# lpiccinelli-eth/UniDepth

Hardware: NVIDIA H100
Metric: images/sec UniDepthV2.infer ViT-L/14 480x640 (higher is better)
Workload: dtype f16 operands, f32 accumulate/residual

## Files before the change

### include/udb.h

```cpp
#ifndef UDB_H_
#define UDB_H_
#include <stddef.h>
#include <stdint.h>

#ifdef __cplusplus
extern "C" {
#endif

#define UDB_VERSION 1

int udb_version(void);

typedef struct udb_profile_entry_t {
  char name[48];
  float ms;
  double flops;
  double bytes;
} udb_profile_entry_t;
int udb_profile_begin(void* stream);
int udb_profile_end(udb_profile_entry_t* out, int32_t cap);
const char* udb_last_error(void);
int64_t udb_launch_count(void);

enum { UDB_A_MATRIX = 0, UDB_A_CONV3X3 = 1 };
// ... 5 lines not shown
  const void* w;
  int32_t M, N, K;
  int32_t lda, ldw;
  int32_t a_mode;
  int32_t conv_B, conv_H, conv_W, conv_C, conv_inH, conv_inW, conv_off, conv_TH, conv_TW;
  int32_t conv_cstride, conv_coff;
  const float* bias;
  const float* gamma;
  const void* resid;
  int32_t resid_f32;
  void* out;
  int32_t out_f32;
  void* out2;
  int32_t out2_leaky;
  int32_t act;
  int32_t store_mode;
  int64_t ldc;
  int32_t rows_per_group, group_stride, row_offset;
  int32_t resid_mod, resid_row_offset;
  int64_t ldr;
  int32_t ct_k, ct_cout, ct_h, ct_w, ct_pad;
  const float* head_w;
  float head_b, head_add;
  int32_t a_split_k;
  int32_t out_split;
  float* ln_stats_out;
  const float* ln_stats_in;
  const float* ln_c1;
  int32_t ln_parts, ln_part_cols;
  float ln_eps;
} udb_gemm_t;

int udb_gemm_f16(const udb_gemm_t* g, void* stream);

typedef struct udb_conv_halo_t {
  const void* x;
  const void* w;
  const float* bias;
  int32_t B, H, W, C, cstride, coff, cout, act;
  void* out;
  int64_t ldc;
  const float* head_w;
  float head_b, head_add;
  float* head_out;
} udb_conv_halo_t;
int udb_conv3x3_halo_f16(const udb_conv_halo_t* c, void* stream);

typedef struct udb_attn_t {
  const void* q;
  const void* k;
  const void* v;
  void* out;
  int32_t B, heads, seq_q, seq_k, head_dim;
  int32_t ldq, ldk, ldv, ldo;
  int32_t q_col0, k_col0, v_col0, o_col0;
  float scale;
  int32_t split;
  int32_t lo_off_q, lo_off_k, lo_off_v, lo_off_o;
} udb_attn_t;

int udb_attention_f16(const udb_attn_t* a, void* stream);

typedef struct udb_layernorm_t {
  const void* in;
  int32_t in_f32;
  void* out;
// ... 292 lines not shown
```

### unidepth_b200/_cabi.py

```python
from __future__ import annotations

import ctypes as C
import os

_HERE = os.path.dirname(os.path.abspath(__file__))
LIB_PATH = os.environ.get("UDB_LIB", os.path.join(_HERE, "libudb.so"))

A_MATRIX, A_CONV3X3 = 0, 1
ACT_NONE, ACT_GELU, ACT_LEAKY = 0, 1, 2
STORE_ROWS, STORE_CONVT, STORE_CONVTILE, STORE_HEAD = 0, 1, 2, 3

vp, i32, i64, f32 = C.c_void_p, C.c_int32, C.c_int64, C.c_float


class Gemm(C.Structure):
    _fields_ = [
        ("a", vp), ("w", vp), ("M", i32), ("N", i32), ("K", i32), ("lda", i32), ("ldw", i32),
        ("a_mode", i32),
        ("conv_B", i32), ("conv_H", i32), ("conv_W", i32), ("conv_C", i32), ("conv_inH", i32),
        ("conv_inW", i32), ("conv_off", i32), ("conv_TH", i32), ("conv_TW", i32),
        ("conv_cstride", i32), ("conv_coff", i32),
        ("bias", vp), ("gamma", vp), ("resid", vp), ("resid_f32", i32), ("out", vp), ("out_f32", i32),
        ("out2", vp), ("out2_leaky", i32), ("act", i32), ("store_mode", i32), ("ldc", i64),
        ("rows_per_group", i32), ("group_stride", i32), ("row_offset", i32),
# ... 125 lines not shown
        ("mean", vp), ("k4", vp), ("B", i32), ("net_h", i32), ("net_w", i32), ("pad_l", i32), ("pad_r", i32),
        ("pad_t", i32), ("pad_b", i32), ("H", i32), ("W", i32), ("out_depth", vp), ("out_points", vp),
    ]


class V1Config(C.Structure):
    _fields_ = [
        ("depths", i32 * 4), ("dims", i32 * 4), ("hidden", i32), ("heads", i32), ("expansion", i32),
        ("dec_depths", i32 * 3), ("encoder", i32), ("net_h", i32), ("net_w", i32),
    ]


class InferV1Args(C.Structure):
    _fields_ = [
        ("rgb", vp), ("rgb_is_u8", i32), ("scale255", i32), ("normalize", i32), ("B", i32), ("H", i32), ("W", i32),
        ("intrinsics", vp), ("skip_camera", i32), ("workspace", vp), ("workspace_bytes", C.c_size_t),
        ("out_intrinsics", vp), ("out_points", vp), ("out_depth", vp),
    ]


class ProfileEntry(C.Structure):
    _fields_ = [("name", C.c_char * 48), ("ms", f32), ("flops", C.c_double), ("bytes", C.c_double)]


DT_F16, DT_F32 = 0, 1

EXPORTS = {
    "udb_version": (i32, []),
    "udb_last_error": (C.c_char_p, []),
    "udb_launch_count": (i64, []),
    "udb_profile_begin": (i32, [vp]),
    "udb_profile_end": (i32, [C.POINTER(ProfileEntry), i32]),
    "udb_gemm_f16": (i32, [C.POINTER(Gemm), vp]),
    "udb_conv3x3_halo_f16": (i32, [C.POINTER(ConvHalo), vp]),
    "udb_attention_f16": (i32, [C.POINTER(Attn), vp]),
    "udb_layernorm": (i32, [C.POINTER(LayerNorm), vp]),
    "udb_preprocess_patchify": (i32, [C.POINTER(Preprocess), vp]),
    "udb_posembed_bicubic": (i32, [vp, i32, i32, vp, i32, i32, vp]),
    "udb_set_cls_rows": (i32, [vp, vp, vp, i32, i32, i32, vp]),
    "udb_set_cls_rows_ln": (i32, [vp, vp, vp, vp, vp, i32, i32, i32, i32, i32, vp]),
    "udb_small_linear_f32": (i32, [C.POINTER(SmallLinear), vp]),
    "udb_camera_attn4_f32": (i32, [vp, vp, vp, vp, i32, i32, i32, vp]),
    "udb_camera_intrinsics": (i32, [vp, i32, i32, i32, f32, i32, i32, vp, vp, vp, vp]),
    "udb_ray_embed": (i32, [C.POINTER(RayEmbed), vp]),
    "udb_upsample2x_nhwc_f16": (i32, [vp, vp, i32, i32, i32, i32, vp]),
    "udb_resize_ac_pad_nhwc_f16": (i32, [vp, vp, i32, i32, i32, i32, i32, i32, i32, vp]),
    "udb_reflect_pad1_nhwc_f16": (i32, [vp, vp, i32, i32, i32, i32, vp]),
    "udb_reflect_border_fill_nhwc_f16": (i32, [vp, i32, i32, i32, i32, vp]),
    "udb_postprocess": (i32, [C.POINTER(Postprocess), vp]),
    "udb_camera_adjust_k": (i32, [vp, i32, f32, i32, i32, vp, vp]),
    "udb_create": (i32, [C.POINTER(Config), C.POINTER(vp)]),
    "udb_destroy": (None, [vp]),
    "udb_set_weight": (i32, [vp, C.c_char_p, vp, C.POINTER(i64), i32, i32]),
    "udb_set_scalar": (i32, [vp, C.c_char_p, C.c_double]),
    "udb_geometry": (i32, [vp, i32, i32, i32, C.POINTER(Geometry)]),
    "udb_workspace_bytes": (C.c_size_t, [vp, i32, i32, i32, i32]),
    "udb_schedule_bytes": (C.c_size_t, [vp, i32, i32, i32, i32]),
    "udb_infer_v2": (i32, [vp, C.POINTER(InferArgs), vp]),
    "udb_v1_preprocess": (i32, [C.POINTER(V1Preprocess), vp]),
    "udb_layernorm_any": (i32, [C.POINTER(LayerNormAny), vp]),
    "udb_dwconv7_nhwc_f16": (i32, [vp, vp, vp, vp, i32, i32, i32, i32, vp]),
    "udb_max_accum_f16": (i32, [vp, vp, i64, i32, vp]),
    "udb_spatial_mean_f32": (i32, [vp, vp, i32, i32, i32, vp]),
    "udb_vit_tap": (i32, [vp, vp, vp, i32, i32, i32, i32, vp]),
    "udb_aa_resize_nhwc_f16": (i32, [vp, vp, i32, i32, i32, i32, i32, i32, vp]),
    "udb_v1_rays_sh81": (i32, [C.POINTER(V1Rays), vp]),
# ... 68 lines not shown
```

### unidepth_b200/csrc/common.cu

```cuda
#include "common.h"

#include <stdarg.h>
#include <stdlib.h>
#include <string.h>

#include <vector>

namespace udb {

static thread_local char g_err[512] = "";
std::atomic<int64_t> g_launches{0};

void set_error(const char* fmt, ...) {
  va_list ap;
  va_start(ap, fmt);
  vsnprintf(g_err, sizeof(g_err), fmt, ap);
  va_end(ap);
}

struct ProfEntry {
  const char* name;
  cudaEvent_t ev;
  double flops, bytes;
};
// ... 34 lines not shown
    per_dev[dev & 63].store(n, std::memory_order_relaxed);
  }
  return n;
}

bool pdl_enabled() {
  static const bool on = [] {
    const char* e = getenv("UDB_PDL");
    return e ? atoi(e) != 0 : true;
  }();
  return on;
}

typedef CUresult (*EncodeTiledFn)(CUtensorMap*, CUtensorMapDataType, cuuint32_t, void*,
                                  const cuuint64_t*, const cuuint64_t*, const cuuint32_t*,
                                  const cuuint32_t*, CUtensorMapInterleave, CUtensorMapSwizzle,
                                  CUtensorMapL2promotion, CUtensorMapFloatOOBfill);

static EncodeTiledFn get_encode() {
  static EncodeTiledFn fn = nullptr;
  if (!fn) {
    void* p = nullptr;
    cudaDriverEntryPointQueryResult q;
    cudaError_t e = cudaGetDriverEntryPoint("cuTensorMapEncodeTiled", &p, cudaEnableDefault, &q);
    if (e != cudaSuccess || q != cudaDriverEntryPointSuccess || !p) {
      set_error("cuTensorMapEncodeTiled entry point unavailable (%s)", cudaGetErrorString(e));
      return nullptr;
    }
    fn = reinterpret_cast<EncodeTiledFn>(p);
  }
  return fn;
}

int make_tmap_f16(CUtensorMap* map, const void* base, int rank, const uint64_t* dims,
                  const uint64_t* strides_bytes, const uint32_t* box, bool swizzle128) {
  EncodeTiledFn fn = get_encode();
  if (!fn) return 1;
  cuuint64_t gdim[5];
  cuuint64_t gstr[5];
  cuuint32_t bx[5];
  cuuint32_t es[5];
  for (int i = 0; i < rank; ++i) {
    gdim[i] = dims[i];
    bx[i] = box[i];
    es[i] = 1;
    if (i > 0) gstr[i - 1] = strides_bytes[i - 1];
  }
  if ((reinterpret_cast<uintptr_t>(base) & 15) != 0) {
    set_error("TMA base pointer %p is not 16-byte aligned", base);
    return 1;
  }
  for (int i = 0; i + 1 < rank; ++i) {
    if (gstr[i] % 16 != 0) {
      set_error("TMA stride %d = %llu bytes is not a multiple of 16", i, (unsigned long long)gstr[i]);
      return 1;
    }
  }
  CUresult r = fn(map, CU_TENSOR_MAP_DATA_TYPE_FLOAT16, (cuuint32_t)rank, const_cast<void*>(base),
                  gdim, gstr, bx, es, CU_TENSOR_MAP_INTERLEAVE_NONE,
                  swizzle128 ? CU_TENSOR_MAP_SWIZZLE_128B : CU_TENSOR_MAP_SWIZZLE_NONE,
                  CU_TENSOR_MAP_L2_PROMOTION_L2_256B, CU_TENSOR_MAP_FLOAT_OOB_FILL_NONE);
  if (r != CUDA_SUCCESS) {
    set_error("cuTensorMapEncodeTiled failed: CUresult %d (rank %d dims %llu,%llu box %u,%u)", (int)r,
              rank, (unsigned long long)dims[0], (unsigned long long)(rank > 1 ? dims[1] : 0), box[0],
              rank > 1 ? box[1] : 0);
    return 1;
  }
  return 0;
}

}

extern "C" {
int udb_version(void) { return UDB_VERSION; }
const char* udb_last_error(void) { return udb::g_err; }
int64_t udb_launch_count(void) { return udb::g_launches.load(); }

int udb_profile_begin(void* stream) {
  using namespace udb;
  if (g_prof_on) { set_error("udb_profile_begin: already profiling"); return 1; }
  g_prof.clear();
  g_prof_stream = reinterpret_cast<cudaStream_t>(stream);
  if (cudaEventCreate(&g_prof_start) != cudaSuccess || cudaEventRecord(g_prof_start, g_prof_stream) != cudaSuccess) {
    set_error("udb_profile_begin: event creation failed");
    return 1;
  }
  g_prof_on = true;
  return 0;
}

int udb_profile_end(udb_profile_entry_t* out, int32_t cap) {
  using namespace udb;
  if (!g_prof_on) { set_error("udb_profile_end: not profiling"); return -1; }
  g_prof_on = false;
// ... 24 lines not shown
```

### unidepth_b200/csrc/common.h

```cpp
#pragma once
#include <cuda.h>
#include <cuda_runtime.h>
#include <stdint.h>
#include <stdio.h>

#include <atomic>

#include "../../include/udb.h"

namespace udb {

void set_error(const char* fmt, ...);
extern std::atomic<int64_t> g_launches;

int check_launch(const char* what);
void note_work(double flops, double bytes);

int num_sms();

inline bool first_on_device(std::atomic<uint64_t>& mask) {
  int d = 0;
  cudaGetDevice(&d);
  const uint64_t bit = 1ull << (d & 63);
  return !(mask.fetch_or(bit) & bit);
}

bool pdl_enabled();

template <typename Kernel, typename... Args>
inline cudaError_t launch_ex(Kernel kernel, dim3 grid, dim3 block, size_t smem, cudaStream_t st, int cluster_x,
                             Args... args) {
  cudaLaunchConfig_t cfg{};
  cfg.gridDim = grid;
  cfg.blockDim = block;
  cfg.dynamicSmemBytes = smem;
  cfg.stream = st;
  cudaLaunchAttribute attr[2];
  int n = 0;
  if (cluster_x > 1) {
    attr[n].id = cudaLaunchAttributeClusterDimension;
    attr[n].val.clusterDim.x = cluster_x;
    attr[n].val.clusterDim.y = 1;
    attr[n].val.clusterDim.z = 1;
    ++n;
  }
  if (pdl_enabled()) {
    attr[n].id = cudaLaunchAttributeProgrammaticStreamSerialization;
    attr[n].val.programmaticStreamSerializationAllowed = 1;
    ++n;
  }
  cfg.attrs = attr;
  cfg.numAttrs = n;
  return cudaLaunchKernelEx(&cfg, kernel, args...);
}

int make_tmap_f16(CUtensorMap* map, const void* base, int rank, const uint64_t* dims,
                  const uint64_t* strides_bytes, const uint32_t* box, bool swizzle128);

}
```

### unidepth_b200/csrc/gemm.cu

```cuda
#include "common.h"
#include "ptx.cuh"

namespace udb {

constexpr int BM = 128;
constexpr int BK = 64;
constexpr int kEpiWarps = 8;
constexpr int kTP = 36;
constexpr int kThreads = (kEpiWarps + 4) * 32;

struct GemmArgs {
  int M, N, K, num_kb;
  int tiles_m, tiles_n;
  int a_mode;
  int conv_B, conv_H, conv_W, conv_cpb , conv_off, conv_TH, conv_TW, conv_tx, conv_ty;
  const float* bias;
  const float* gamma;
  const void* resid;
  int resid_f32;
  void* out;
  int out_f32;
  __half* out2;
  int out2_leaky;
  int act;
  int store_mode;
  long long ldc, ldr;
  int rpg, gstride, roff;
  int resid_mod, resid_roff;
  int ct_k, ct_cout, ct_h, ct_w, ct_pad;
  int conv_coff;
  const float* head_w;
  float head_b, head_add;
  int a_wrap;
  int out_split;
  float* stats_out;
  const float* ln_stats;
  const float* ln_c1;
  int ln_parts, ln_part_cols;
  float ln_eps;
};

template <int BN>
struct GemmCfg {
  static constexpr int kStages = BN >= 256 ? 3 : (BN >= 192 ? 4 : (BN >= 128 ? 5 : 7));
  static constexpr int kABytes = BM * BK * 2;
  static constexpr int kBBytes = BN * BK * 2;
  static constexpr int kStageBytes = kABytes + kBBytes;
  static constexpr int kStagingBytes = kEpiWarps * (32 * kTP * 4 + 2 * 32 * 4);
  static constexpr int kSmemBytes = kStages * kStageBytes + kStagingBytes + 256 ;
  static_assert(kSmemBytes <= 232448, "shared memory per block");
};

struct EpiWarp {
  float* T;
  float* Twg;
  uint32_t* roff_out;
  uint32_t* roff_res;
  int wg, wq, grp, lane, r_in_tile;
};

template <int BN, bool LNF>
__device__ __forceinline__ void epilogue_tile(const GemmArgs& p, const EpiWarp& w, const float (&acc)[BN / 2], const int mt,
                                              const int nt) {
  constexpr int kGroups = BN >= 64 ? 2 : 1;
  constexpr int kColsPerGrp = BN / kGroups;
  const int grp = w.grp, lane = w.lane, r_in_tile = w.r_in_tile;
  const bool active = grp < kGroups;
  float* T = w.T;
  uint32_t* roff_out = w.roff_out;
  uint32_t* roff_res = w.roff_res;
  bool valid = false;
  long long out_off = 0, res_off = 0;
  uint32_t vmask = 0;
  float ln_mean = 0.f, ln_rstd = 1.f;
  float st_pivot = 0.f, st_s1 = 0.f, st_s2 = 0.f;
  bool st_first = true;
  if (active) {

    const int m = mt * BM + r_in_tile;
    if (p.store_mode == UDB_STORE_CONVTILE || p.store_mode == UDB_STORE_HEAD) {
      const int per_img = p.conv_tx * p.conv_ty;
      const int b = mt / per_img;
      const int r = mt % per_img;
      const int y = (r / p.conv_tx) * p.conv_TH + r_in_tile / p.conv_TW;
// ... 51 lines not shown
    }
    bar_sync(1 + w.wg, 128);
    if (!active) continue;
    const int col = grp * kColsPerGrp + c;
    const int n0 = nt * BN + col;
    float v[32];
#pragma unroll
    for (int j = 0; j < 32; j += 4) {
      const float4 t = *reinterpret_cast<const float4*>(T + lane * kTP + j);
      v[j] = t.x; v[j + 1] = t.y; v[j + 2] = t.z; v[j + 3] = t.w;
    }
    __syncwarp();
    if (n0 >= p.N) continue;
    if (LNF && p.ln_stats) {
      const float4* cp = reinterpret_cast<const float4*>(p.ln_c1 + n0);
      const float mr = ln_mean * ln_rstd;
#pragma unroll
      for (int j = 0; j < 8; ++j) {
        const float4 c4 = __ldg(cp + j);
        v[4 * j] = fmaf(v[4 * j], ln_rstd, -mr * c4.x);
        v[4 * j + 1] = fmaf(v[4 * j + 1], ln_rstd, -mr * c4.y);
        v[4 * j + 2] = fmaf(v[4 * j + 2], ln_rstd, -mr * c4.z);
        v[4 * j + 3] = fmaf(v[4 * j + 3], ln_rstd, -mr * c4.w);
      }
    }
    if (p.bias) {
      const float4* bp = reinterpret_cast<const float4*>(p.bias + n0);
#pragma unroll
      for (int j = 0; j < 8; ++j) {
        const float4 b4 = __ldg(bp + j);
        v[4 * j] += b4.x; v[4 * j + 1] += b4.y; v[4 * j + 2] += b4.z; v[4 * j + 3] += b4.w;
      }
    }
    if (p.act == UDB_ACT_GELU) {
#pragma unroll
      for (int j = 0; j < 32; j += 2) gelu_erf_pair(v[j], v[j + 1]);
    } else if (p.act == UDB_ACT_LEAKY) {
#pragma unroll
      for (int j = 0; j < 32; ++j) v[j] = leaky(v[j]);
    }
    if (p.store_mode == UDB_STORE_HEAD) {
      float head = p.head_b;
#pragma unroll
      for (int j = 0; j < 32; ++j) head = fmaf(v[j], __ldg(p.head_w + j), head);
      head = fminf(fmaxf(head, -8.0f), 8.0f) + p.head_add;
      if (valid) reinterpret_cast<float*>(p.out)[out_off] = expf(head);
      continue;
    }
    if (p.gamma) {
      const float4* gp = reinterpret_cast<const float4*>(p.gamma + n0);
#pragma unroll
      for (int j = 0; j < 8; ++j) {
        const float4 g4 = __ldg(gp + j);
        v[4 * j] *= g4.x; v[4 * j + 1] *= g4.y; v[4 * j + 2] *= g4.z; v[4 * j + 3] *= g4.w;
      }
    }
    long long coff = n0;
    if (p.store_mode == UDB_STORE_CONVT) {
      const int tap = n0 / p.ct_cout;
      const int co = n0 % p.ct_cout;
      const long long W2 = (long long)p.ct_w * p.ct_k + 2 * p.ct_pad;
      coff = ((long long)(tap / p.ct_k) * W2 + (tap % p.ct_k)) * p.ct_cout + co;
    }
    const uint32_t c32 = static_cast<uint32_t>(coff);
    const int l4 = (lane & 7) * 4, rq = lane >> 3;
    float* Trow = T + lane * kTP;
    auto stage_rows = [&](const float (&x)[32]) {
#pragma unroll
      for (int j = 0; j < 32; j += 4)
        *reinterpret_cast<float4*>(Trow + j) = make_float4(x[j], x[j + 1], x[j + 2], x[j + 3]);
    };
    auto for_rows = [&](auto&& body) {
      if (vmask == 0xffffffffu) {
// ... 72 lines not shown
                  make_uint2(pack_half2(t.x - h01.x, t.y - h01.y), pack_half2(t.z - h23.x, t.w - h23.y));
            }
          });
        }
      }
      __syncwarp();
    }
    if (p.out2) {
      if (p.out2_leaky) {
#pragma unroll
        for (int j = 0; j < 32; ++j) v[j] = leaky(v[j]);
        stage_rows(v);
      } else if (!p.out) {
        stage_rows(v);
      }
      __syncwarp();
      __half* op = p.out2 + c32 + l4;
      for_rows([&](int rr, bool ok) {
        const float4 t = *reinterpret_cast<const float4*>(T + rr * kTP + l4);
        if (ok) *reinterpret_cast<uint2*>(op + roff_out[rr]) = make_uint2(pack_half2(t.x, t.y), pack_half2(t.z, t.w));
      });
      __syncwarp();
    }
  }
  if (LNF && p.stats_out && active && valid && !st_first) {
    const float n = (float)kColsPerGrp;
    const float mean_p = st_pivot + st_s1 / n;
    const float m2_p = fmaxf(st_s2 - st_s1 * st_s1 / n, 0.f);
    const long long orow = out_off / p.ldc;
    reinterpret_cast<float2*>(p.stats_out)[orow * (p.tiles_n * kGroups) + nt * kGroups + grp] = make_float2(mean_p, m2_p);
  }
}

template <int BN, bool LNF>
__global__ void __launch_bounds__(kThreads, 1)
gemm_f16_kernel(const __grid_constant__ CUtensorMap tmA, const __grid_constant__ CUtensorMap tmB,
                const GemmArgs p) {
  using Cfg = GemmCfg<BN>;
  constexpr int kStages = Cfg::kStages;
  extern __shared__ __align__(1024) uint8_t smem[];
  uint8_t* sA = smem;
  uint8_t* sB = smem + kStages * Cfg::kABytes;
  uint8_t* staging = smem + kStages * Cfg::kStageBytes;
  uint64_t* bars = reinterpret_cast<uint64_t*>(staging + Cfg::kStagingBytes);
  uint64_t* full_bar = bars;
  uint64_t* empty_bar = bars + kStages;

  const int warp = threadIdx.x >> 5;
  const int lane = threadIdx.x & 31;
  pdl_launch_dependents();

  if (threadIdx.x == 0) {
    if (smem_u32(smem) & 1023) __trap();
    prefetch_tmap(&tmA);
    prefetch_tmap(&tmB);
    for (int i = 0; i < kStages; ++i) {
      mbar_init(&full_bar[i], 1);
      mbar_init(&empty_bar[i], kEpiWarps);
    }
    fence_barrier_init();
  }
  __syncthreads();
  pdl_wait();

  const int num_tiles = p.tiles_m * p.tiles_n;

  if (warp >= kEpiWarps) {
    setmaxnreg_dec<40>();
    if (warp != kEpiWarps) return;
    const bool elected = elect_one();
    int stage = 0;
    uint32_t phase = 0;
    for (int tile = blockIdx.x; tile < num_tiles; tile += gridDim.x) {
      const int mt = tile / p.tiles_n;
      const int nt = tile % p.tiles_n;
      int cb = 0, cy = 0, cx = 0;
      if (p.a_mode == UDB_A_CONV3X3) {
        const int per_img = p.conv_tx * p.conv_ty;
        cb = mt / per_img;
        const int r = mt % per_img;
        cy = (r / p.conv_tx) * p.conv_TH + p.conv_off;
        cx = (r % p.conv_tx) * p.conv_TW + p.conv_off;
      }
      for (int kb = 0; kb < p.num_kb; ++kb) {
        mbar_wait(&empty_bar[stage], phase ^ 1);
        if (elected) {
          mbar_arrive_expect_tx(&full_bar[stage], Cfg::kStageBytes);
          if (p.a_mode == UDB_A_CONV3X3) {
            const int tap = kb / p.conv_cpb;
            const int c0 = p.conv_coff + (kb % p.conv_cpb) * BK;
            tma_load_4d(sA + stage * Cfg::kABytes, &tmA, &full_bar[stage], c0, cx + tap % 3, cy + tap / 3, cb);
          } else {
            int ka = kb * BK;
            if (p.a_wrap && ka >= p.a_wrap) ka -= p.a_wrap;
            tma_load_2d(sA + stage * Cfg::kABytes, &tmA, &full_bar[stage], ka, mt * BM);
          }
          tma_load_2d(sB + stage * Cfg::kBBytes, &tmB, &full_bar[stage], kb * BK, nt * BN);
        }
        __syncwarp();
        if (++stage == kStages) {
          stage = 0;
          phase ^= 1;
        }
      }
    }
  } else {
    setmaxnreg_inc<232>();
    const int wg = warp >> 2, wq = warp & 3;
    float* Twg = reinterpret_cast<float*>(staging) + wg * 4 * 32 * kTP;
    uint32_t* roff = reinterpret_cast<uint32_t*>(staging + kEpiWarps * 32 * kTP * 4) + warp * 64;
    const EpiWarp ctx{Twg + wq * 32 * kTP, Twg, roff, roff + 32, wg, wq, wq >> 1, lane, 64 * wg + 32 * (wq & 1) + lane};
    float acc[BN / 2];
#pragma unroll
    for (int i = 0; i < BN / 2; ++i) acc[i] = 0.f;
    int stage = 0;
    uint32_t phase = 0;
    for (int tile = blockIdx.x; tile < num_tiles; tile += gridDim.x) {
      const int mt = tile / p.tiles_n;
      const int nt = tile % p.tiles_n;
      int prev = -1;
      for (int kb = 0; kb < p.num_kb; ++kb) {
        mbar_wait(&full_bar[stage], phase);
        const uint64_t da = gmma_desc_sw128(smem_u32(sA + stage * Cfg::kABytes + wg * 64 * 128), 16, 1024);
        const uint64_t db = gmma_desc_sw128(smem_u32(sB + stage * Cfg::kBBytes), 16, 1024);
        wgmma_fence();
#pragma unroll
        for (int k = 0; k < BK / 16; ++k) WgmmaSS<BN>::run(acc, da + 2 * k, db + 2 * k, (kb | k) != 0 ? 1u : 0u);
        wgmma_commit();
        wgmma_wait<1>();
        if (prev >= 0 && lane == 0) mbar_arrive(&empty_bar[prev]);
        prev = stage;
        if (++stage == kStages) {
          stage = 0;
          phase ^= 1;
        }
      }
      wgmma_wait<0>();
      wgmma_fence_regs(acc);
      if (prev >= 0 && lane == 0) mbar_arrive(&empty_bar[prev]);
      epilogue_tile<BN, LNF>(p, ctx, acc, mt, nt);
    }
  }
}

template <int BN, bool LNF>
static int launch_gemm(const CUtensorMap& tmA, const CUtensorMap& tmB, const GemmArgs& a, cudaStream_t st) {
  using Cfg = GemmCfg<BN>;
  static std::atomic<uint64_t> attr_mask{0};
  if (first_on_device(attr_mask)) {
    cudaError_t e = cudaFuncSetAttribute(gemm_f16_kernel<BN, LNF>, cudaFuncAttributeMaxDynamicSharedMemorySize,
                                         Cfg::kSmemBytes);
    if (e != cudaSuccess) {
      set_error("gemm: cudaFuncSetAttribute(%d B smem): %s", Cfg::kSmemBytes, cudaGetErrorString(e));
      return 1;
    }
  }
  const int tiles = a.tiles_m * a.tiles_n;
  const int grid = tiles < num_sms() ? tiles : num_sms();
  cudaError_t e = launch_ex(gemm_f16_kernel<BN, LNF>, dim3(grid), dim3(kThreads), Cfg::kSmemBytes, st, 1, tmA, tmB, a);
  if (e != cudaSuccess) {
    set_error("gemm_f16_kernel launch: %s", cudaGetErrorString(e));
    return 1;
  }
  return check_launch("gemm_f16_kernel");
}

static bool aligned(const void* p, uintptr_t bytes) { return (reinterpret_cast<uintptr_t>(p) & (bytes - 1)) == 0; }

static int check_gemm_layout(const udb_gemm_t* g) {
  const int sm = g->store_mode;
  if (g->M < 1 || g->N < 1 || g->K < 1) { set_error("udb_gemm_f16: M=%d N=%d K=%d must be >= 1", g->M, g->N, g->K); return 1; }
  if (sm < UDB_STORE_ROWS || sm > UDB_STORE_HEAD) { set_error("udb_gemm_f16: unknown store_mode %d", sm); return 1; }
  const long long ldr = g->ldr > 0 ? g->ldr : g->ldc;
  if (sm == UDB_STORE_HEAD) {
    if (!g->out || !g->out_f32 || !aligned(g->out, 4)) { set_error("udb_gemm_f16: HEAD store needs a 4-byte aligned f32 `out`"); return 1; }
    if (!g->head_w || !aligned(g->head_w, 16)) { set_error("udb_gemm_f16: `head_w` must be non-null and 16-byte aligned"); return 1; }
  } else {
    if (g->out && !aligned(g->out, g->out_f32 ? 16 : 8)) {
      set_error("udb_gemm_f16: `out` %p must be %d-byte aligned", g->out, g->out_f32 ? 16 : 8); return 1;
    }
    if (g->out2 && !aligned(g->out2, 8)) { set_error("udb_gemm_f16: `out2` %p must be 8-byte aligned", g->out2); return 1; }
    if (g->resid && !aligned(g->resid, g->resid_f32 ? 16 : 8)) {
      set_error("udb_gemm_f16: `resid` %p must be %d-byte aligned", g->resid, g->resid_f32 ? 16 : 8); return 1;
    }
    if (sm != UDB_STORE_CONVT) {
      if ((g->out || g->out2) && (g->ldc < 1 || g->ldc % 4)) { set_error("udb_gemm_f16: `ldc`=%lld must be a positive multiple of 4", (long long)g->ldc); return 1; }
      if (g->resid && (ldr < 1 || ldr % 4)) { set_error("udb_gemm_f16: `ldr`=%lld must be a positive multiple of 4", ldr); return 1; }
      if ((g->out || g->out2) && g->ldc < (long long)g->N + g->out_split) {
        set_error("udb_gemm_f16: `ldc`=%lld < N + out_split = %lld: rows would overlap", (long long)g->ldc, (long long)g->N + g->out_split);
        return 1;
      }
      if (g->resid && ldr < g->N) { set_error("udb_gemm_f16: `ldr`=%lld < N=%d: residual rows would overlap", ldr, g->N); return 1; }
// ... 28 lines not shown
    if (g->ct_k < 1 || g->ct_h < 1 || g->ct_w < 1 || g->ct_pad < 0 || g->ct_cout < 1) {
      set_error("udb_gemm_f16: CONVT geometry `ct_k`=%d `ct_h`=%d `ct_w`=%d `ct_pad`=%d `ct_cout`=%d", g->ct_k, g->ct_h, g->ct_w, g->ct_pad,
                g->ct_cout);
      return 1;
    }
    if (g->N != g->ct_k * g->ct_k * g->ct_cout) { set_error("udb_gemm_f16: CONVT needs N == ct_k^2 * ct_cout (N=%d)", g->N); return 1; }
    const long long m = g->M - 1, hw = (long long)g->ct_h * g->ct_w, b = m / hw, r = m % hw, y = r / g->ct_w, x = r % g->ct_w;
    const long long W2 = (long long)g->ct_w * g->ct_k + 2 * g->ct_pad, H2 = (long long)g->ct_h * g->ct_k + 2 * g->ct_pad;
    out_row = res_row = ((b * H2 + y * g->ct_k + g->ct_pad) * W2 + x * g->ct_k + g->ct_pad) * g->ct_cout;
  } else {
    if (g->conv_B < 1 || g->conv_H < 1 || g->conv_W < 1) {
      set_error("udb_gemm_f16: conv_B=%d conv_H=%d conv_W=%d must be >= 1", g->conv_B, g->conv_H, g->conv_W); return 1;
    }
    const long long last_px = (long long)g->conv_B * g->conv_H * g->conv_W - 1;
    out_row = last_px * g->ldc;
    res_row = last_px * ldr;
  }
  const long long lim = 1ll << 32;
  if ((g->out || g->out2) && out_row >= lim) { set_error("udb_gemm_f16: `out` row offset %lld exceeds 2^32 elements", out_row); return 1; }
  if (g->resid && res_row >= lim) { set_error("udb_gemm_f16: `resid` row offset %lld exceeds 2^32 elements", res_row); return 1; }

  if (g->a_mode == UDB_A_CONV3X3) {
    const int pad = g->conv_off == 0 ? 2 : (g->conv_off == -1 ? 0 : -1);
    if (pad < 0) { set_error("udb_gemm_f16: `conv_off`=%d must be 0 (prepadded) or -1 (zero padding)", g->conv_off); return 1; }
    if (g->conv_inH != g->conv_H + pad || g->conv_inW != g->conv_W + pad) {
      set_error("udb_gemm_f16: `conv_inH`x`conv_inW` = %dx%d must be %dx%d for conv_off %d", g->conv_inH, g->conv_inW, g->conv_H + pad,
                g->conv_W + pad, g->conv_off);
      return 1;
    }
  }
  return 0;
}

}

extern "C" int udb_gemm_f16(const udb_gemm_t* g, void* stream) {
  using namespace udb;
  if (!g || !g->a || !g->w) { set_error("udb_gemm_f16: null operand"); return 1; }
  if (g->N % 32 != 0) { set_error("udb_gemm_f16: N=%d must be a multiple of 32", g->N); return 1; }
  if (check_gemm_layout(g)) return 1;
  GemmArgs a{};
  a.M = g->M; a.N = g->N; a.K = g->K;
  a.num_kb = (g->K + BK - 1) / BK;
  a.a_mode = g->a_mode;
  a.bias = g->bias; a.gamma = g->gamma; a.resid = g->resid; a.resid_f32 = g->resid_f32;
  a.out = g->out; a.out_f32 = g->out_f32; a.out2 = reinterpret_cast<__half*>(g->out2); a.out2_leaky = g->out2_leaky;
  a.act = g->act; a.store_mode = g->store_mode;
  a.ldc = g->ldc; a.ldr = g->ldr > 0 ? g->ldr : g->ldc;
  a.rpg = g->rows_per_group; a.gstride = g->group_stride; a.roff = g->row_offset;
  a.resid_mod = g->resid_mod; a.resid_roff = g->resid_row_offset;
  a.ct_k = g->ct_k; a.ct_cout = g->ct_cout; a.ct_h = g->ct_h; a.ct_w = g->ct_w; a.ct_pad = g->ct_pad;
  a.conv_coff = g->conv_coff;
  a.head_w = g->head_w; a.head_b = g->head_b; a.head_add = g->head_add;
  a.a_wrap = 0;
  a.out_split = g->out_split;
  if (g->a_split_k > 0) {
    if (g->a_mode != UDB_A_MATRIX || g->a_split_k % BK || g->K != 3 * g->a_split_k || g->lda < 2 * g->a_split_k) {
      set_error("udb_gemm_f16: split operands need a_mode MATRIX, K1 %% 64 == 0, K == 3*K1, lda >= 2*K1 (K1=%d K=%d lda=%d)",
                g->a_split_k, g->K, g->lda);
      return 1;
    }
    a.a_wrap = 2 * g->a_split_k;
  }
  a.stats_out = g->ln_stats_out; a.ln_stats = g->ln_stats_in; a.ln_c1 = g->ln_c1; a.ln_eps = g->ln_eps;
  a.ln_parts = g->ln_parts; a.ln_part_cols = g->ln_part_cols;
  if ((g->ln_stats_out || g->ln_stats_in) && g->store_mode != UDB_STORE_ROWS) {
    set_error("udb_gemm_f16: fused LayerNorm statistics need the ROWS store"); return 1;
// ... 38 lines not shown
    }
    const int TH = g->conv_TH > 0 ? g->conv_TH : 8, TW = g->conv_TW > 0 ? g->conv_TW : 16;
    if (TH * TW != BM) { set_error("udb_gemm_f16: conv tile %dx%d != 128 pixels", TH, TW); return 1; }
    a.conv_B = g->conv_B; a.conv_H = g->conv_H; a.conv_W = g->conv_W; a.conv_cpb = g->conv_C / BK; a.conv_off = g->conv_off;
    a.conv_TH = TH; a.conv_TW = TW;
    a.conv_tx = (g->conv_W + TW - 1) / TW; a.conv_ty = (g->conv_H + TH - 1) / TH;
    a.tiles_m = g->conv_B * a.conv_tx * a.conv_ty;
    a.M = a.tiles_m * BM;
    const uint64_t cs = g->conv_cstride > 0 ? g->conv_cstride : g->conv_C;
    if ((uint64_t)g->conv_coff + g->conv_C > cs || (g->conv_coff % 8)) {
      set_error("udb_gemm_f16: bad conv channel slice (off %d, C %d, stride %d)", g->conv_coff, g->conv_C, (int)cs);
      return 1;
    }
    const uint64_t dims[4] = {cs, (uint64_t)g->conv_inW, (uint64_t)g->conv_inH, (uint64_t)g->conv_B};
    const uint64_t str[3] = {cs * 2, (uint64_t)g->conv_inW * cs * 2, (uint64_t)g->conv_inH * g->conv_inW * cs * 2};
    const uint32_t box[4] = {(uint32_t)BK, (uint32_t)TW, (uint32_t)TH, 1};
    if (make_tmap_f16(&tmA, g->a, 4, dims, str, box, true)) return 1;
  } else {
    a.tiles_m = (g->M + BM - 1) / BM;
    if (g->store_mode == UDB_STORE_CONVTILE || g->store_mode == UDB_STORE_HEAD) {
      set_error("udb_gemm_f16: tile store modes need a_mode == CONV3X3"); return 1;
    }
    const uint64_t dims[2] = {(uint64_t)(g->a_split_k > 0 ? 2 * g->a_split_k : g->K), (uint64_t)g->M};
    const uint64_t str[1] = {(uint64_t)g->lda * 2};
    const uint32_t box[2] = {(uint32_t)BK, (uint32_t)BM};
    if (make_tmap_f16(&tmA, g->a, 2, dims, str, box, true)) return 1;
  }
  {
    const uint64_t dims[2] = {(uint64_t)g->K, (uint64_t)g->N};
    const uint64_t str[1] = {(uint64_t)g->ldw * 2};
    const uint32_t box[2] = {(uint32_t)BK, (uint32_t)bn};
    if (make_tmap_f16(&tmB, g->w, 2, dims, str, box, true)) return 1;
  }
  cudaStream_t st = reinterpret_cast<cudaStream_t>(stream);
  note_work(2.0 * a.M * (double)g->N * g->K,
            2.0 * ((double)a.M * (g->a_mode == UDB_A_CONV3X3 ? g->conv_C : (g->a_split_k ? 2 * g->a_split_k : g->K)) + (double)g->N * g->K) +
                (double)a.M * g->N * ((g->out ? (g->out_f32 ? 4 : 2) : 0) + (g->out2 ? 2 : 0) + (g->resid ? (g->resid_f32 ? 4 : 2) : 0)));
  const bool lnf = g->ln_stats_out || g->ln_stats_in;
  if (lnf) {
    switch (bn) {
      case 256: return launch_gemm<256, true>(tmA, tmB, a, st);
      case 192: return launch_gemm<192, true>(tmA, tmB, a, st);
      case 128: return launch_gemm<128, true>(tmA, tmB, a, st);
      case 64: return launch_gemm<64, true>(tmA, tmB, a, st);
      default: return launch_gemm<32, true>(tmA, tmB, a, st);
    }
  }
  switch (bn) {
    case 256: return launch_gemm<256, false>(tmA, tmB, a, st);
    case 192: return launch_gemm<192, false>(tmA, tmB, a, st);
    case 128: return launch_gemm<128, false>(tmA, tmB, a, st);
    case 64: return launch_gemm<64, false>(tmA, tmB, a, st);
    default: return launch_gemm<32, false>(tmA, tmB, a, st);
  }
}
```

### unidepth_b200/csrc/ptx.cuh

```cuda
#pragma once
#include <cuda_fp16.h>
#include <cuda_runtime.h>
#include <stdint.h>
#include <stdio.h>

namespace udb {

__device__ __forceinline__ uint32_t smem_u32(const void* p) {
  return static_cast<uint32_t>(__cvta_generic_to_shared(p));
}

__device__ __forceinline__ bool elect_one() {
  uint32_t pred = 0;
  asm volatile(
      "{\n\t"
      ".reg .b32 rx;\n\t"
      ".reg .pred px;\n\t"
      "elect.sync rx|px, 0xffffffff;\n\t"
      "selp.b32 %0, 1, 0, px;\n\t"
      "}\n"
      : "=r"(pred));
  return pred != 0;
}

// ... 40 lines not shown
  }
}

__device__ __forceinline__ void fence_proxy_async_smem() {
  asm volatile("fence.proxy.async.shared::cta;" ::: "memory");
}

__device__ __forceinline__ void prefetch_tmap(const void* tmap) {
  asm volatile("prefetch.tensormap [%0];" ::"l"(reinterpret_cast<uint64_t>(tmap)) : "memory");
}
__device__ __forceinline__ void tma_load_2d(void* smem_dst, const void* tmap, uint64_t* bar, int c0,
                                            int c1) {
  asm volatile(
      "cp.async.bulk.tensor.2d.shared::cluster.global.mbarrier::complete_tx::bytes"
      " [%0], [%1, {%3, %4}], [%2];" ::"r"(smem_u32(smem_dst)),
      "l"(reinterpret_cast<uint64_t>(tmap)), "r"(smem_u32(bar)), "r"(c0), "r"(c1)
      : "memory");
}
__device__ __forceinline__ void tma_load_3d(void* smem_dst, const void* tmap, uint64_t* bar, int c0,
                                            int c1, int c2) {
  asm volatile(
      "cp.async.bulk.tensor.3d.shared::cluster.global.mbarrier::complete_tx::bytes"
      " [%0], [%1, {%3, %4, %5}], [%2];" ::"r"(smem_u32(smem_dst)),
      "l"(reinterpret_cast<uint64_t>(tmap)), "r"(smem_u32(bar)), "r"(c0), "r"(c1), "r"(c2)
      : "memory");
}
__device__ __forceinline__ void tma_load_4d(void* smem_dst, const void* tmap, uint64_t* bar, int c0,
                                            int c1, int c2, int c3) {
  asm volatile(
      "cp.async.bulk.tensor.4d.shared::cluster.global.mbarrier::complete_tx::bytes"
      " [%0], [%1, {%3, %4, %5, %6}], [%2];" ::"r"(smem_u32(smem_dst)),
      "l"(reinterpret_cast<uint64_t>(tmap)), "r"(smem_u32(bar)), "r"(c0), "r"(c1), "r"(c2), "r"(c3)
      : "memory");
}


__device__ __forceinline__ void wgmma_fence() { asm volatile("wgmma.fence.sync.aligned;" ::: "memory"); }
__device__ __forceinline__ void wgmma_commit() { asm volatile("wgmma.commit_group.sync.aligned;" ::: "memory"); }
template <int N>
__device__ __forceinline__ void wgmma_wait() {
  asm volatile("wgmma.wait_group.sync.aligned %0;" ::"n"(N) : "memory");
}
template <int R>
__device__ __forceinline__ void wgmma_fence_regs(float (&d)[R]) {
#pragma unroll
  for (int i = 0; i < R; ++i) asm volatile("" : "+f"(d[i])::"memory");
}
template <uint32_t R>
__device__ __forceinline__ void setmaxnreg_inc() { asm volatile("setmaxnreg.inc.sync.aligned.u32 %0;" ::"n"(R)); }
template <uint32_t R>
__device__ __forceinline__ void setmaxnreg_dec() { asm volatile("setmaxnreg.dec.sync.aligned.u32 %0;" ::"n"(R)); }
__device__ __forceinline__ void bar_sync(int id, int threads) {
  asm volatile("bar.sync %0, %1;" ::"r"(id), "r"(threads) : "memory");
}

__device__ __forceinline__ uint64_t gmma_desc_sw128(uint32_t smem_addr, uint32_t lbo_bytes, uint32_t sbo_bytes) {
  uint64_t d = 0;
  d |= static_cast<uint64_t>((smem_addr & 0x3FFFF) >> 4);
  d |= static_cast<uint64_t>((lbo_bytes >> 4) & 0x3FFF) << 16;
  d |= static_cast<uint64_t>((sbo_bytes >> 4) & 0x3FFF) << 32;
  d |= static_cast<uint64_t>(1) << 62;
  return d;
}

__device__ __forceinline__ void wgmma_ss_n32(float (&d)[16], uint64_t da, uint64_t db, uint32_t scale_d) {
  asm volatile(
// ... 123 lines not shown
```

Baseline: 216.9.

## Add TMA-based GEMM epilogue with TMA residual prefetch and swizzled smem staging

```diff
diff --git a/include/udb.h b/include/udb.h
--- a/include/udb.h
+++ b/include/udb.h
@@ -61,6 +61,7 @@
 } udb_gemm_t;
 
 int udb_gemm_f16(const udb_gemm_t* g, void* stream);
+int udb_gemm_tma_epilogue_used(void);
 
 typedef struct udb_conv_halo_t {
   const void* x;
diff --git a/unidepth_b200/_cabi.py b/unidepth_b200/_cabi.py
--- a/unidepth_b200/_cabi.py
+++ b/unidepth_b200/_cabi.py
@@ -181,6 +181,7 @@
     "udb_profile_begin": (i32, [vp]),
     "udb_profile_end": (i32, [C.POINTER(ProfileEntry), i32]),
     "udb_gemm_f16": (i32, [C.POINTER(Gemm), vp]),
+    "udb_gemm_tma_epilogue_used": (i32, []),
     "udb_conv3x3_halo_f16": (i32, [C.POINTER(ConvHalo), vp]),
     "udb_attention_f16": (i32, [C.POINTER(Attn), vp]),
     "udb_layernorm": (i32, [C.POINTER(LayerNorm), vp]),
diff --git a/unidepth_b200/csrc/common.cu b/unidepth_b200/csrc/common.cu
--- a/unidepth_b200/csrc/common.cu
+++ b/unidepth_b200/csrc/common.cu
@@ -90,8 +90,8 @@
   return fn;
 }
 
-int make_tmap_f16(CUtensorMap* map, const void* base, int rank, const uint64_t* dims,
-                  const uint64_t* strides_bytes, const uint32_t* box, bool swizzle128) {
+int make_tmap(CUtensorMap* map, const void* base, int rank, const uint64_t* dims, const uint64_t* strides_bytes,
+              const uint32_t* box, CUtensorMapDataType dtype, CUtensorMapSwizzle swizzle) {
   EncodeTiledFn fn = get_encode();
   if (!fn) return 1;
   cuuint64_t gdim[5];
@@ -114,10 +114,9 @@
       return 1;
     }
   }
-  CUresult r = fn(map, CU_TENSOR_MAP_DATA_TYPE_FLOAT16, (cuuint32_t)rank, const_cast<void*>(base),
-                  gdim, gstr, bx, es, CU_TENSOR_MAP_INTERLEAVE_NONE,
-                  swizzle128 ? CU_TENSOR_MAP_SWIZZLE_128B : CU_TENSOR_MAP_SWIZZLE_NONE,
-                  CU_TENSOR_MAP_L2_PROMOTION_L2_256B, CU_TENSOR_MAP_FLOAT_OOB_FILL_NONE);
+  CUresult r = fn(map, dtype, (cuuint32_t)rank, const_cast<void*>(base), gdim, gstr, bx, es,
+                  CU_TENSOR_MAP_INTERLEAVE_NONE, swizzle, CU_TENSOR_MAP_L2_PROMOTION_L2_256B,
+                  CU_TENSOR_MAP_FLOAT_OOB_FILL_NONE);
   if (r != CUDA_SUCCESS) {
     set_error("cuTensorMapEncodeTiled failed: CUresult %d (rank %d dims %llu,%llu box %u,%u)", (int)r,
               rank, (unsigned long long)dims[0], (unsigned long long)(rank > 1 ? dims[1] : 0), box[0],
diff --git a/unidepth_b200/csrc/common.h b/unidepth_b200/csrc/common.h
--- a/unidepth_b200/csrc/common.h
+++ b/unidepth_b200/csrc/common.h
@@ -54,7 +54,12 @@
   return cudaLaunchKernelEx(&cfg, kernel, args...);
 }
 
-int make_tmap_f16(CUtensorMap* map, const void* base, int rank, const uint64_t* dims,
-                  const uint64_t* strides_bytes, const uint32_t* box, bool swizzle128);
+int make_tmap(CUtensorMap* map, const void* base, int rank, const uint64_t* dims, const uint64_t* strides_bytes,
+              const uint32_t* box, CUtensorMapDataType dtype, CUtensorMapSwizzle swizzle);
+inline int make_tmap_f16(CUtensorMap* map, const void* base, int rank, const uint64_t* dims,
+                         const uint64_t* strides_bytes, const uint32_t* box, bool swizzle128) {
+  return make_tmap(map, base, rank, dims, strides_bytes, box, CU_TENSOR_MAP_DATA_TYPE_FLOAT16,
+                   swizzle128 ? CU_TENSOR_MAP_SWIZZLE_128B : CU_TENSOR_MAP_SWIZZLE_NONE);
+}
 
 }
diff --git a/unidepth_b200/csrc/gemm.cu b/unidepth_b200/csrc/gemm.cu
--- a/unidepth_b200/csrc/gemm.cu
+++ b/unidepth_b200/csrc/gemm.cu
@@ -1,3 +1,6 @@
+#include <stdlib.h>
+#include <string.h>
+
 #include "common.h"
 #include "ptx.cuh"
 
@@ -40,16 +43,31 @@
   float ln_eps;
 };
 
-template <int BN>
+constexpr int kEpiBox = 64 * 32 * 4;
+
+template <int BN, bool TMAE = false>
 struct GemmCfg {
-  static constexpr int kStages = BN >= 256 ? 3 : (BN >= 192 ? 4 : (BN >= 128 ? 5 : 7));
+  static constexpr int kStages = TMAE ? (BN >= 192 ? 4 : (BN >= 128 ? 6 : 8))
+                                      : (BN >= 256 ? 3 : (BN >= 192 ? 4 : (BN >= 128 ? 5 : 7)));
   static constexpr int kABytes = BM * BK * 2;
   static constexpr int kBBytes = BN * BK * 2;
   static constexpr int kStageBytes = kABytes + kBBytes;
-  static constexpr int kStagingBytes = kEpiWarps * (32 * kTP * 4 + 2 * 32 * 4);
+  static constexpr int kStagingBytes = TMAE ? 2 * 2 * kEpiBox : kEpiWarps * (32 * kTP * 4 + 2 * 32 * 4);
   static constexpr int kSmemBytes = kStages * kStageBytes + kStagingBytes + 256 ;
   static_assert(kSmemBytes <= 232448, "shared memory per block");
+  static_assert(2 * kStages + 4 <= 32, "barriers");
 };
+
+template <int N>
+__device__ __forceinline__ void apply_act(const int act, float (&v)[N]) {
+  if (act == UDB_ACT_GELU) {
+#pragma unroll
+    for (int j = 0; j < N; j += 2) gelu_erf_pair(v[j], v[j + 1]);
+  } else if (act == UDB_ACT_LEAKY) {
+#pragma unroll
+    for (int j = 0; j < N; ++j) v[j] = leaky(v[j]);
+  }
+}
 
 struct EpiWarp {
   float* T;
@@ -167,13 +185,7 @@
         v[4 * j] += b4.x; v[4 * j + 1] += b4.y; v[4 * j + 2] += b4.z; v[4 * j + 3] += b4.w;
       }
     }
-    if (p.act == UDB_ACT_GELU) {
-#pragma unroll
-      for (int j = 0; j < 32; j += 2) gelu_erf_pair(v[j], v[j + 1]);
-    } else if (p.act == UDB_ACT_LEAKY) {
-#pragma unroll
-      for (int j = 0; j < 32; ++j) v[j] = leaky(v[j]);
-    }
+    apply_act(p.act, v);
     if (p.store_mode == UDB_STORE_HEAD) {
       float head = p.head_b;
 #pragma unroll
@@ -312,11 +324,95 @@
   }
 }
 
-template <int BN, bool LNF>
+struct EpiTma {
+  uint8_t* buf;
+  uint64_t* full;
+  uint64_t* empty;
+  uint32_t chunk;
+};
+
+template <int BN>
+__device__ __forceinline__ void epilogue_tile_tma(const GemmArgs& p, const CUtensorMap* tmC, EpiTma& e,
+                                                  const float (&acc)[BN / 2], const int mt, const int nt, const int wg,
+                                                  const int wq, const int lane) {
+  const bool leader = wq == 0 && lane == 0;
+  const int q = lane & 3, rr = lane >> 2;
+  const bool has_res = p.resid != nullptr;
+  const int row0 = mt * BM + 64 * wg;
+#pragma unroll
+  for (int c = 0; c < BN / 32; ++c, ++e.chunk) {
+    const int b = e.chunk & 1;
+    uint8_t* box = e.buf + (2 * b + wg) * kEpiBox;
+    if (has_res) {
+      mbar_wait(&e.full[b], (e.chunk >> 1) & 1);
+    } else {
+      if (leader) bulk_wait_read<1>();
+      bar_sync(1 + wg, 128);
+    }
+    const int n0 = nt * BN + 32 * c;
+    float v[16];
+#pragma unroll
+    for (int j = 0; j < 16; ++j) v[j] = acc[16 * c + j];
+    if (p.bias) {
+#pragma unroll
+      for (int j = 0; j < 4; ++j) {
+        const float2 b2 = __ldg(reinterpret_cast<const float2*>(p.bias + n0 + 8 * j + 2 * q));
+        v[4 * j] += b2.x; v[4 * j + 1] += b2.y; v[4 * j + 2] += b2.x; v[4 * j + 3] += b2.y;
+      }
+    }
+    apply_act(p.act, v);
+    if (p.gamma) {
+#pragma unroll
+      for (int j = 0; j < 4; ++j) {
+        const float2 g2 = __ldg(reinterpret_cast<const float2*>(p.gamma + n0 + 8 * j + 2 * q));
+        v[4 * j] *= g2.x; v[4 * j + 1] *= g2.y; v[4 * j + 2] *= g2.x; v[4 * j + 3] *= g2.y;
+      }
+    }
+    if (p.out_f32) {
+#pragma unroll
+      for (int j = 0; j < 4; ++j) {
+#pragma unroll
+        for (int h = 0; h < 2; ++h) {
+          const int r = 16 * wq + rr + 8 * h;
+          float2* s = reinterpret_cast<float2*>(box + r * 128 + (((2 * j + (q >> 1)) ^ rr) << 4) + 8 * (q & 1));
+          float x0 = v[4 * j + 2 * h], x1 = v[4 * j + 2 * h + 1];
+          if (has_res) {
+            const float2 t = *s;
+            x0 += t.x; x1 += t.y;
+          }
+          *s = make_float2(x0, x1);
+        }
+      }
+    } else {
+#pragma unroll
+      for (int j = 0; j < 4; ++j) {
+#pragma unroll
+        for (int h = 0; h < 2; ++h) {
+          const int r = 16 * wq + rr + 8 * h;
+          *reinterpret_cast<uint32_t*>(box + r * 64 + ((j ^ ((r >> 1) & 3)) << 4) + 4 * q) =
+              pack_half2(v[4 * j + 2 * h], v[4 * j + 2 * h + 1]);
+        }
+      }
+    }
+    fence_proxy_async_smem();
+    bar_sync(1 + wg, 128);
+    if (leader) {
+      if (row0 < p.M) tma_store_2d(tmC, box, n0, row0);
+      bulk_commit();
+      if (has_res) {
+        bulk_wait_read<0>();
+        mbar_arrive(&e.empty[b]);
+      }
+    }
+  }
+}
+
+template <int BN, bool LNF, bool TMAE>
 __global__ void __launch_bounds__(kThreads, 1)
 gemm_f16_kernel(const __grid_constant__ CUtensorMap tmA, const __grid_constant__ CUtensorMap tmB,
-                const GemmArgs p) {
-  using Cfg = GemmCfg<BN>;
+                const __grid_constant__ CUtensorMap tmC, const __grid_constant__ CUtensorMap tmR, const GemmArgs p) {
+  static_assert(!(TMAE && LNF), "the TMA epilogue carries no fused-LayerNorm code");
+  using Cfg = GemmCfg<BN, TMAE>;
   constexpr int kStages = Cfg::kStages;
   extern __shared__ __align__(1024) uint8_t smem[];
   uint8_t* sA = smem;
@@ -325,6 +421,8 @@
   uint64_t* bars = reinterpret_cast<uint64_t*>(staging + Cfg::kStagingBytes);
   uint64_t* full_bar = bars;
   uint64_t* empty_bar = bars + kStages;
+  uint64_t* epi_full = bars + 2 * kStages;
+  uint64_t* epi_empty = epi_full + 2;
 
   const int warp = threadIdx.x >> 5;
   const int lane = threadIdx.x & 31;
@@ -338,6 +436,14 @@
       mbar_init(&full_bar[i], 1);
       mbar_init(&empty_bar[i], kEpiWarps);
     }
+    if constexpr (TMAE) {
+      prefetch_tmap(&tmC);
+      if (p.resid) prefetch_tmap(&tmR);
+      for (int i = 0; i < 2; ++i) {
+        mbar_init(&epi_full[i], 1);
+        mbar_init(&epi_empty[i], 2);
+      }
+    }
     fence_barrier_init();
   }
   __syncthreads();
@@ -347,6 +453,25 @@
 
   if (warp >= kEpiWarps) {
     setmaxnreg_dec<40>();
+    if constexpr (TMAE) {
+      if (warp == kEpiWarps + 1 && p.resid) {
+        const bool elected = elect_one();
+        uint32_t chunk = 0;
+        for (int tile = blockIdx.x; tile < num_tiles; tile += gridDim.x) {
+          const int mt = tile / p.tiles_n;
+          const int nt = tile % p.tiles_n;
+          for (int c = 0; c < BN / 32; ++c, ++chunk) {
+            const int b = chunk & 1;
+            mbar_wait(&epi_empty[b], ((chunk >> 1) & 1) ^ 1);
+            if (elected) {
+              mbar_arrive_expect_tx(&epi_full[b], 2 * kEpiBox);
+              tma_load_2d(staging + 2 * b * kEpiBox, &tmR, &epi_full[b], nt * BN + 32 * c, mt * BM);
+            }
+            __syncwarp();
+          }
+        }
+      }
+    }
     if (warp != kEpiWarps) return;
     const bool elected = elect_one();
     int stage = 0;
@@ -390,6 +515,7 @@
     float* Twg = reinterpret_cast<float*>(staging) + wg * 4 * 32 * kTP;
     uint32_t* roff = reinterpret_cast<uint32_t*>(staging + kEpiWarps * 32 * kTP * 4) + warp * 64;
     const EpiWarp ctx{Twg + wq * 32 * kTP, Twg, roff, roff + 32, wg, wq, wq >> 1, lane, 64 * wg + 32 * (wq & 1) + lane};
+    EpiTma etma{staging, epi_full, epi_empty, 0};
     float acc[BN / 2];
 #pragma unroll
     for (int i = 0; i < BN / 2; ++i) acc[i] = 0.f;
@@ -418,17 +544,22 @@
       wgmma_wait<0>();
       wgmma_fence_regs(acc);
       if (prev >= 0 && lane == 0) mbar_arrive(&empty_bar[prev]);
-      epilogue_tile<BN, LNF>(p, ctx, acc, mt, nt);
+      if constexpr (TMAE) epilogue_tile_tma<BN>(p, &tmC, etma, acc, mt, nt, wg, wq, lane);
+      else epilogue_tile<BN, LNF>(p, ctx, acc, mt, nt);
+    }
+    if constexpr (TMAE) {
+      if (wq == 0 && lane == 0) bulk_wait<0>();
     }
   }
 }
 
-template <int BN, bool LNF>
-static int launch_gemm(const CUtensorMap& tmA, const CUtensorMap& tmB, const GemmArgs& a, cudaStream_t st) {
-  using Cfg = GemmCfg<BN>;
+template <int BN, bool LNF, bool TMAE>
+static int launch_gemm(const CUtensorMap& tmA, const CUtensorMap& tmB, const CUtensorMap& tmC, const CUtensorMap& tmR,
+                       const GemmArgs& a, cudaStream_t st) {
+  using Cfg = GemmCfg<BN, TMAE>;
   static std::atomic<uint64_t> attr_mask{0};
   if (first_on_device(attr_mask)) {
-    cudaError_t e = cudaFuncSetAttribute(gemm_f16_kernel<BN, LNF>, cudaFuncAttributeMaxDynamicSharedMemorySize,
+    cudaError_t e = cudaFuncSetAttribute(gemm_f16_kernel<BN, LNF, TMAE>, cudaFuncAttributeMaxDynamicSharedMemorySize,
                                          Cfg::kSmemBytes);
     if (e != cudaSuccess) {
       set_error("gemm: cudaFuncSetAttribute(%d B smem): %s", Cfg::kSmemBytes, cudaGetErrorString(e));
@@ -437,7 +568,8 @@
   }
   const int tiles = a.tiles_m * a.tiles_n;
   const int grid = tiles < num_sms() ? tiles : num_sms();
-  cudaError_t e = launch_ex(gemm_f16_kernel<BN, LNF>, dim3(grid), dim3(kThreads), Cfg::kSmemBytes, st, 1, tmA, tmB, a);
+  cudaError_t e = launch_ex(gemm_f16_kernel<BN, LNF, TMAE>, dim3(grid), dim3(kThreads), Cfg::kSmemBytes, st, 1, tmA, tmB, tmC,
+                            tmR, a);
   if (e != cudaSuccess) {
     set_error("gemm_f16_kernel launch: %s", cudaGetErrorString(e));
     return 1;
@@ -532,7 +664,21 @@
   return 0;
 }
 
+static bool tma_epilogue_ok(const udb_gemm_t* g) {
+  const char* env = getenv("UDB_GEMM_TMA_EPILOGUE");
+  if (env && atoi(env) == 0) return false;
+  if (g->store_mode != UDB_STORE_ROWS || g->a_mode != UDB_A_MATRIX || g->rows_per_group > 0 || g->resid_mod > 0) return false;
+  if (g->out_split || g->out2 || g->ln_stats_out || g->ln_stats_in || !g->out) return false;
+  if (!aligned(g->out, 16) || (g->ldc * (g->out_f32 ? 4 : 2)) % 16) return false;
+  const long long ldr = g->ldr > 0 ? g->ldr : g->ldc;
+  return !g->resid || (g->resid_f32 && g->out_f32 && aligned(g->resid, 16) && (ldr * 4) % 16 == 0);
 }
+
+static thread_local int g_last_tma_epilogue = 0;
+
+}
+
+extern "C" int udb_gemm_tma_epilogue_used(void) { return udb::g_last_tma_epilogue; }
 
 extern "C" int udb_gemm_f16(const udb_gemm_t* g, void* stream) {
   using namespace udb;
@@ -637,6 +783,24 @@
     const uint32_t box[2] = {(uint32_t)BK, (uint32_t)bn};
     if (make_tmap_f16(&tmB, g->w, 2, dims, str, box, true)) return 1;
   }
+  const bool tmae = tma_epilogue_ok(g);
+  CUtensorMap tmC, tmR;
+  memset(&tmC, 0, sizeof(tmC));
+  memset(&tmR, 0, sizeof(tmR));
+  if (tmae) {
+    const uint64_t dims[2] = {(uint64_t)g->N, (uint64_t)g->M};
+    const uint64_t str_c[1] = {(uint64_t)g->ldc * (g->out_f32 ? 4 : 2)};
+    const uint32_t box_c[2] = {32, 64};
+    if (make_tmap(&tmC, g->out, 2, dims, str_c, box_c, g->out_f32 ? CU_TENSOR_MAP_DATA_TYPE_FLOAT32 : CU_TENSOR_MAP_DATA_TYPE_FLOAT16,
+                  g->out_f32 ? CU_TENSOR_MAP_SWIZZLE_128B : CU_TENSOR_MAP_SWIZZLE_64B))
+      return 1;
+    if (g->resid) {
+      const uint64_t str_r[1] = {(uint64_t)a.ldr * 4};
+      const uint32_t box_r[2] = {32, BM};
+      if (make_tmap(&tmR, g->resid, 2, dims, str_r, box_r, CU_TENSOR_MAP_DATA_TYPE_FLOAT32, CU_TENSOR_MAP_SWIZZLE_128B)) return 1;
+    }
+  }
+  g_last_tma_epilogue = tmae ? 1 : 0;
   cudaStream_t st = reinterpret_cast<cudaStream_t>(stream);
   note_work(2.0 * a.M * (double)g->N * g->K,
             2.0 * ((double)a.M * (g->a_mode == UDB_A_CONV3X3 ? g->conv_C : (g->a_split_k ? 2 * g->a_split_k : g->K)) + (double)g->N * g->K) +
@@ -644,18 +808,27 @@
   const bool lnf = g->ln_stats_out || g->ln_stats_in;
   if (lnf) {
     switch (bn) {
-      case 256: return launch_gemm<256, true>(tmA, tmB, a, st);
-      case 192: return launch_gemm<192, true>(tmA, tmB, a, st);
-      case 128: return launch_gemm<128, true>(tmA, tmB, a, st);
-      case 64: return launch_gemm<64, true>(tmA, tmB, a, st);
-      default: return launch_gemm<32, true>(tmA, tmB, a, st);
+      case 256: return launch_gemm<256, true, false>(tmA, tmB, tmC, tmR, a, st);
+      case 192: return launch_gemm<192, true, false>(tmA, tmB, tmC, tmR, a, st);
+      case 128: return launch_gemm<128, true, false>(tmA, tmB, tmC, tmR, a, st);
+      case 64: return launch_gemm<64, true, false>(tmA, tmB, tmC, tmR, a, st);
+      default: return launch_gemm<32, true, false>(tmA, tmB, tmC, tmR, a, st);
+    }
+  }
+  if (tmae) {
+    switch (bn) {
+      case 256: return launch_gemm<256, false, true>(tmA, tmB, tmC, tmR, a, st);
+      case 192: return launch_gemm<192, false, true>(tmA, tmB, tmC, tmR, a, st);
+      case 128: return launch_gemm<128, false, true>(tmA, tmB, tmC, tmR, a, st);
+      case 64: return launch_gemm<64, false, true>(tmA, tmB, tmC, tmR, a, st);
+      default: return launch_gemm<32, false, true>(tmA, tmB, tmC, tmR, a, st);
     }
   }
   switch (bn) {
-    case 256: return launch_gemm<256, false>(tmA, tmB, a, st);
-    case 192: return launch_gemm<192, false>(tmA, tmB, a, st);
-    case 128: return launch_gemm<128, false>(tmA, tmB, a, st);
-    case 64: return launch_gemm<64, false>(tmA, tmB, a, st);
-    default: return launch_gemm<32, false>(tmA, tmB, a, st);
+    case 256: return launch_gemm<256, false, false>(tmA, tmB, tmC, tmR, a, st);
+    case 192: return launch_gemm<192, false, false>(tmA, tmB, tmC, tmR, a, st);
+    case 128: return launch_gemm<128, false, false>(tmA, tmB, tmC, tmR, a, st);
+    case 64: return launch_gemm<64, false, false>(tmA, tmB, tmC, tmR, a, st);
+    default: return launch_gemm<32, false, false>(tmA, tmB, tmC, tmR, a, st);
   }
 }
diff --git a/unidepth_b200/csrc/ptx.cuh b/unidepth_b200/csrc/ptx.cuh
--- a/unidepth_b200/csrc/ptx.cuh
+++ b/unidepth_b200/csrc/ptx.cuh
@@ -96,6 +96,21 @@
       " [%0], [%1, {%3, %4, %5, %6}], [%2];" ::"r"(smem_u32(smem_dst)),
       "l"(reinterpret_cast<uint64_t>(tmap)), "r"(smem_u32(bar)), "r"(c0), "r"(c1), "r"(c2), "r"(c3)
       : "memory");
+}
+__device__ __forceinline__ void tma_store_2d(const void* tmap, const void* smem_src, int c0, int c1) {
+  asm volatile(
+      "cp.async.bulk.tensor.2d.global.shared::cta.bulk_group [%0, {%2, %3}], [%1];" ::"l"(reinterpret_cast<uint64_t>(tmap)),
+      "r"(smem_u32(smem_src)), "r"(c0), "r"(c1)
+      : "memory");
+}
+__device__ __forceinline__ void bulk_commit() { asm volatile("cp.async.bulk.commit_group;" ::: "memory"); }
+template <int N>
+__device__ __forceinline__ void bulk_wait_read() {
+  asm volatile("cp.async.bulk.wait_group.read %0;" ::"n"(N) : "memory");
+}
+template <int N>
+__device__ __forceinline__ void bulk_wait() {
+  asm volatile("cp.async.bulk.wait_group %0;" ::"n"(N) : "memory");
 }
 
 
```

Result: faster. 231.7, median of 6 (+6.8%).
